# ankitkumar93/compute-war

Measured on AMD Instinct MI355X. Metric: GB/s ingested (Skein-512 + LZ4, 64 KiB blocks), higher is better.
Workload: dtype u64; 1 GPU; skein512+lz4, 1048576 x 65536 B uniform-random blocks/GPU in HBM; blocks_per_gpu=1048576, block_bytes=65536, parallelism=block-sharded x1, gather-only RCCL

## Files before the change

### compute_war_amd/csrc/cw_api.hip

```cpp

#include <hip/hip_runtime.h>

#include <atomic>
#include <condition_variable>
#include <cstdarg>
#include <cstdio>
#include <cstdlib>
#include <cstring>
#include <deque>
#include <memory>
#include <mutex>
#include <string>
#include <thread>
#include <vector>

#include "../../include/cw_hashcompress.h"
#include "cw_device.h"
#include "stream_scratch.h"

namespace {

thread_local char t_err[512] = "";

int fail(int code, const char *fmt, ...)
// ... 104 lines not shown
            HIP_TRY(hipStreamCreateWithFlags(&stream, hipStreamNonBlocking));
        }
        HIP_TRY(side.open(cw::SideStream::least, borrowed ? lender->side.stream : nullptr));
        HIP_TRY(hipEventCreateWithFlags(&ev_meta, hipEventDisableTiming));
        HIP_TRY(hipEventCreateWithFlags(&ev_payload, hipEventDisableTiming));
        HIP_TRY(hipEventCreateWithFlags(&ev_h2d, hipEventDisableTiming));
        return CW_OK;
    }
    void release()
    {
        src.release(); dst.release(); pack.release(); sizes.release(); offs.release(); dig.release();
        h_src.release(); h_meta.release(); h_pack.release();
        if (stream && !borrowed) { cw::release_stream_workspaces(stream); (void)hipStreamDestroy(stream); }
        if (side.stream && !side.borrowed) cw::release_stream_workspaces(side.stream);
        side.release();
        borrowed = false;
        if (ev_meta) (void)hipEventDestroy(ev_meta);
        if (ev_payload) (void)hipEventDestroy(ev_payload);
        if (ev_h2d) (void)hipEventDestroy(ev_h2d);
        stream = nullptr; ev_meta = ev_payload = ev_h2d = nullptr;
    }
};

struct FusedHint { uint32_t *h_queued = nullptr; hipEvent_t ev = nullptr; bool pending = false; size_t blocks_of_copy = 0; float queued_share = 0.f; };

struct ThreadCtx {
    int device = -1;
    FusedHint hint;
    hipStream_t stream = nullptr;
    hipStream_t s_h2d = nullptr, s_d2h = nullptr;
    cw::SideStream side;
    DevBuf src, dst, dig, sizes;
    Slot slot[kSlots];
    int open(int dev)
    {
        if (stream) return CW_OK;
        device = dev;
        HIP_TRY(hipSetDevice(dev));
        HIP_TRY(hipStreamCreateWithFlags(&stream, hipStreamNonBlocking));
        HIP_TRY(hipStreamCreateWithFlags(&s_h2d, hipStreamNonBlocking));
        HIP_TRY(hipStreamCreateWithFlags(&s_d2h, hipStreamNonBlocking));
        HIP_TRY(side.open(cw::SideStream::least));
        return CW_OK;
    }
    ~ThreadCtx()
    {
        if (!stream) return;
        (void)hipSetDevice(device);
        src.release(); dst.release(); dig.release(); sizes.release();
        for (Slot &s : slot) s.release();
        if (hint.ev) (void)hipEventDestroy(hint.ev);
        if (hint.h_queued) (void)hipHostFree(hint.h_queued);
        cw::release_stream_workspaces(side.stream); cw::release_stream_workspaces(stream);
        side.release();
        (void)hipStreamDestroy(s_h2d); (void)hipStreamDestroy(s_d2h); (void)hipStreamDestroy(stream);
    }
};
struct ThreadCtxSet { std::unique_ptr<ThreadCtx> of[kMaxDevices]; };
thread_local ThreadCtxSet t_ctxs;

int thread_ctx(ThreadCtx **out)
{
    int rc = ensure_init();
    if (rc != CW_OK) return rc;
    const int d = current_device();
    std::unique_ptr<ThreadCtx> &c = t_ctxs.of[d];
    if (!c) c.reset(new ThreadCtx);
    if ((rc = c->open(d)) != CW_OK) return rc;
    *out = c.get();
    return CW_OK;
}

const size_t kMaxChunkBytes = (size_t)256 << 20;

// ... 58 lines not shown
void positive(int &f, const char *v) { if (atoi(v) > 0) f = atoi(v); }
void positive(long &f, const char *v) { if (atol(v) > 0) f = atol(v); }

struct KnobDef { const char *name; void (*decode)(Knobs &k, const char *v); };
const KnobDef kKnobTable[] = {
    {"CW_SKEIN_SLICED", [](Knobs &k, const char *v) { k.skein_sliced = v[0] != '0'; }},
    {"CW_LZ4_LANES_FP", [](Knobs &k, const char *v) { k.lz4_lanes_fp = v[0] != '0'; }},
    {"CW_LZF_STHREAD", [](Knobs &k, const char *v) { k.lzf_sthread = v[0] != '0'; }},
    {"CW_SERIAL", [](Knobs &k, const char *v) { k.serial = v[0] == '1'; }},
    {"CW_DEBUG_HOST", [](Knobs &k, const char *v) { k.debug_host = v[0] == '1'; }},
    {"CW_PREPARE_COLD", [](Knobs &k, const char *v) { k.prepare_cold = v[0] == '1'; }},
    {"CW_FUSED_GATE", [](Knobs &k, const char *v) { k.fused_gate = v[0] == '1'; }},
    {"CW_HOST_SHARED_STREAMS", [](Knobs &k, const char *v) { k.host_shared_streams = v[0] == '1'; }},
    {"CW_LANES_CONCURRENT", [](Knobs &k, const char *v) { k.lanes_concurrent = v[0] != '0'; }},
    {"CW_SIDE_PRIO", [](Knobs &k, const char *v) { k.side_prio = v[0] == '0' ? cw::SidePrio::none : v[0] == '2' ? cw::SidePrio::both : cw::SidePrio::lanes; }},
    {"CW_LZ4_MODE", [](Knobs &k, const char *v) {
         k.lz4_mode = !strcmp(v, "scan") ? cw::Lz4Mode::scan : !strcmp(v, "generic") ? cw::Lz4Mode::generic
                    : !strcmp(v, "stream") ? cw::Lz4Mode::stream : !strcmp(v, "cut") ? cw::Lz4Mode::cut : cw::Lz4Mode::normal; }},
    {"CW_LZF_MODE", [](Knobs &k, const char *v) { k.lzf_mode = !strcmp(v, "cut") ? cw::LzfMode::cut : !strcmp(v, "table") ? cw::LzfMode::table : cw::LzfMode::normal; }},
    {"CW_SKEIN_MODE", [](Knobs &k, const char *v) { k.skein_mode = !strcmp(v, "steps") ? cw::SkeinMode::steps : cw::SkeinMode::lines; }},
    {"CW_LZ4_PARSE", [](Knobs &k, const char *v) { k.lz4_parse_fp = !strcmp(v, "fp"); }},
    {"CW_DEBUG_LZF", [](Knobs &k, const char *) { k.debug_lzf = true; }},
    {"CW_SCAN_WPC", [](Knobs &k, const char *v) { positive(k.scan_wpc, v); }},
    {"CW_PARSE_WPC", [](Knobs &k, const char *v) { positive(k.parse_wpc, v); }},
    {"CW_LANES_WPC", [](Knobs &k, const char *v) { positive(k.lanes_wpc, v); }},
    {"CW_LANES_RESERVE", [](Knobs &k, const char *v) { positive(k.lanes_reserve, v); }},
    {"CW_VTAB_WPC", [](Knobs &k, const char *v) { positive(k.vtab_wpc, v); }},
    {"CW_LZF_ST_WPC", [](Knobs &k, const char *v) { positive(k.lzf_st_wpc, v); }},
    {"CW_LZF_ROUND", [](Knobs &k, const char *v) { positive(k.lzf_round, v); }},
    {"CW_LZF_LDS_MAX", [](Knobs &k, const char *v) { positive(k.lzf_lds_max, v); }},
    {"CW_SKEIN_NSLICES", [](Knobs &k, const char *v) { positive(k.skein_nslices, v); }},
    {"CW_HOST_CHUNK_MB", [](Knobs &k, const char *v) { positive(k.host_chunk_mb, v); }},
    {"CW_HOST_BIG_CHUNK_MB", [](Knobs &k, const char *v) { positive(k.host_big_chunk_mb, v); }},
    {"CW_CDC_SEGMENT", [](Knobs &k, const char *v) { positive(k.cdc_segment, v); }},
    {"CW_LZ_FORCE_REDO", [](Knobs &k, const char *v) { k.force_redo = atoi(v) > 0; }},
    {"CW_LZF_SHARE_GIVE_UP", [](Knobs &k, const char *v) { k.lzf_share_give_up = atoi(v) > 0; }},
    {"CW_LZ4_LANES", [](Knobs &k, const char *v) { k.lz4_lanes = atoi(v); }},
    {"CW_LZF_LANES", [](Knobs &k, const char *v) { k.lzf_lanes = atoi(v); }},
    {"CW_DECODE_LANES", [](Knobs &k, const char *v) { k.decode_lanes = atoi(v); }},
    {"CW_LANES_LEAVE", [](Knobs &k, const char *v) { k.lanes_leave = atoi(v); }},
    {"CW_VTAB_MIN", [](Knobs &k, const char *v) { k.vtab_min = atoi(v); }},
    {"CW_VTAB_MAX", [](Knobs &k, const char *v) { k.vtab_max = atoi(v); }},
    {"CW_VTAB_RESERVE", [](Knobs &k, const char *v) { k.vtab_reserve = atoi(v); }},
    {"CW_LZ4_VTAB", [](Knobs &k, const char *v) { k.lz4_vtab = atoi(v); }},
    {"CW_LZ4_LANES_RING", [](Knobs &k, const char *v) { k.lz4_lanes_ring = atoi(v); }},
    {"CW_LZ4_HEADW", [](Knobs &k, const char *v) { k.lz4_headw = atoi(v); }},
// ... 174 lines not shown
    const hipStream_t side = side_s.stream;
    struct Gate { int hash_alg; const uint8_t *src; size_t bb, stride, n; uint8_t *dig; hipStream_t side; cw::SideStream::Fork *fork; int rc; bool called; };
    Gate gate = {hash_alg, d_src, block_bytes, src_stride, nblocks, d_digests, side, &fork, CW_OK, false};
    const cw::AfterScan hook = {[](void *p) -> hipError_t {
                                    Gate *g = static_cast<Gate *>(p);
                                    g->called = true;
                                    g->rc = dev_hash(g->hash_alg, g->src, g->bb, g->stride, g->n, g->dig, g->side, false, true);
                                    return g->rc != CW_OK ? hipErrorUnknown : g->fork->join();
                                }, &gate};
    ThreadCtx *tc = nullptr;
    FusedHint *hint = comp_alg == CW_COMP_LZ4 && thread_ctx(&tc) == CW_OK ? &tc->hint : nullptr;
    if (hint && hint->pending) {
        const hipError_t q = hipEventQuery(hint->ev);
        if (q == hipSuccess) {
            hint->pending = false;
            if (hint->blocks_of_copy) hint->queued_share = (float)*hint->h_queued / (float)hint->blocks_of_copy;
        } else if (q == hipErrorNotReady) {
            (void)hipGetLastError();
        }
    }
    const bool gated = hint && (kn.fused_gate ? *kn.fused_gate : block_bytes <= 4096 && nblocks >= 16384 && hint->queued_share >= 0.25f);
    rc = dev_compress(comp_alg, d_src, block_bytes, src_stride, nblocks, d_dst, dst_stride, d_sizes, main_s, gated ? &hook : nullptr);
    if (gate.called && gate.rc != CW_OK) return gate.rc;
    if (rc == CW_OK && !gate.called) rc = dev_hash(hash_alg, d_src, block_bytes, src_stride, nblocks, d_digests, side, false, true);
    HIP_TRY(fork.join());
    if (rc == CW_OK && hint && !hint->pending) {
        const uint32_t *word = cw::lz4_queued_blocks_word(main_s);
        if (word) {
            if (!hint->h_queued) HIP_TRY(hipHostMalloc(reinterpret_cast<void **>(&hint->h_queued), 64, hipHostMallocDefault));
            if (!hint->ev) HIP_TRY(hipEventCreateWithFlags(&hint->ev, hipEventDisableTiming));
            HIP_TRY(hipMemcpyAsync(hint->h_queued, word, sizeof(uint32_t), hipMemcpyDeviceToHost, main_s));
            HIP_TRY(hipEventRecord(hint->ev, main_s));
            hint->pending = true;
            hint->blocks_of_copy = nblocks;
        }
    }
    return rc;
}

int cw_dev_hash_and_compress(int hash_alg, int comp_alg, const void *d_src, size_t block_bytes, size_t src_stride,
                             size_t nblocks, void *d_digests, void *d_dst, size_t dst_stride, uint32_t *d_sizes, void *stream)
{
    if (comp_alg == CW_COMP_NONE) return cw_dev_hash(hash_alg, d_src, block_bytes, src_stride, nblocks, d_digests, stream);
    if (hash_alg == CW_HASH_NONE)
        return cw_dev_compress(comp_alg, d_src, block_bytes, src_stride, nblocks, d_dst, dst_stride, d_sizes, stream);
    ThreadCtx *c;
    int rc = thread_ctx(&c);
    if (rc != CW_OK) return rc;
    if (nblocks == 0) return CW_OK;
    if (!d_src || !d_dst || !d_sizes || !d_digests) return fail(CW_ERR_BAD_ARG, "NULL device pointer");
    if ((rc = check_block(block_bytes)) != CW_OK) return rc;
    if (src_stride < block_bytes) return fail(CW_ERR_BAD_ARG, "src_stride < block_bytes");
    return dev_fused(c->side, hash_alg, comp_alg, (const uint8_t *)d_src, block_bytes, src_stride, nblocks, (uint8_t *)d_digests, (uint8_t *)d_dst,
                     dst_stride, d_sizes, (hipStream_t)stream);
}

int cw_dev_decompress(int comp_alg, const void *d_comp, size_t comp_stride, const uint32_t *d_sizes, size_t nblocks, void *d_dst,
                      size_t block_bytes, uint32_t *d_status, void *stream)
{
// ... 87 lines not shown
    return CW_OK;
}
int cw_dev_download(void *dst, const void *d_src, size_t bytes)
{
    int rc = ensure_init();
    if (rc != CW_OK) return rc;
    HIP_TRY(hipMemcpy(dst, d_src, bytes, hipMemcpyDeviceToHost));
    return CW_OK;
}
int cw_dev_synchronize(void)
{
    int rc = ensure_init();
    if (rc != CW_OK) return rc;
    HIP_TRY(hipDeviceSynchronize());
    return CW_OK;
}

#ifdef CW_CLOCK_STAMP
int cw_debug_clock_read(int which, unsigned long long *out)
{
    int rc = ensure_init();
    if (rc != CW_OK) return rc;
    HIP_TRY(hipDeviceSynchronize());
    HIP_TRY(which == 0 ? cw::skein_clock_read(out) : cw::lz4_clock_read(out));
    return CW_OK;
}
#endif

void cw_profile_enable(int on) { t_prof_on = on != 0; }

int cw_profile_read(double ms_sum[3], unsigned count[3], int reset)
{
    for (int k = 0; k < PROF_KINDS; k++) { ms_sum[k] = 0; count[k] = 0; }
    for (ProfSpan &p : t_prof) {
        float ms = 0;
        HIP_TRY(hipEventSynchronize(p.b));
        HIP_TRY(hipEventElapsedTime(&ms, p.a, p.b));
        ms_sum[p.kind] += ms;
        count[p.kind]++;
    }
    if (reset) {
        for (ProfSpan &p : t_prof) { (void)hipEventDestroy(p.a); (void)hipEventDestroy(p.b); }
        t_prof.clear();
    }
    return CW_OK;
}

// ... 1102 lines not shown
```

### compute_war_amd/csrc/cw_device.h

```cpp
#pragma once

#include <hip/hip_runtime.h>
#include <stddef.h>
#include <stdint.h>

#include <optional>

#ifndef CW_SKEIN_THREADS
#define CW_SKEIN_THREADS 64
#endif

namespace cw {

#ifdef CW_CLOCK_STAMP
constexpr unsigned kClockSlots = 1024;
struct ClockScope {
    unsigned long long m0 = 0, r0 = 0;
    unsigned long long *rec;
    bool on;
    __device__ ClockScope(unsigned long long *buf, unsigned wg) : rec(buf + 4 * (wg % kClockSlots)), on(threadIdx.x == 0)
    {
        if (on) { m0 = __builtin_amdgcn_s_memtime(); r0 = __builtin_amdgcn_s_memrealtime(); }
    }
    __device__ ~ClockScope()
    {
        if (on) {
            const unsigned long long m1 = __builtin_amdgcn_s_memtime(), r1 = __builtin_amdgcn_s_memrealtime();
            rec[0] = m0; rec[1] = r0; rec[2] = m1; rec[3] = r1;
        }
    }
};
#define CW_CLOCK_SCOPE(buf) ClockScope clock_scope_(buf, blockIdx.x)
#define CW_CLOCK_SCOPE_KEYED(buf, key) ClockScope clock_scope_(buf, ((unsigned)(key) % 8u) * 128u + blockIdx.x % 128u)
hipError_t skein_clock_read(unsigned long long *out);
hipError_t lz4_clock_read(unsigned long long *out);
#else
#define CW_CLOCK_SCOPE(buf) do { } while (0)
#define CW_CLOCK_SCOPE_KEYED(buf, key) do { } while (0)
#endif

struct SkeinIV { uint64_t w[8]; };

void note_kernels(int kind, const char *names);
enum class Lz4Mode : uint8_t { normal, scan, generic, stream, cut };
enum class LzfMode : uint8_t { normal, cut, table };
enum class SkeinMode : uint8_t { by_lean, steps, lines };
enum class SidePrio : uint8_t { both, lanes, none };
struct Knobs {
    bool skein_sliced = true, lz4_lanes_fp = true, lzf_sthread = true;
    bool serial = false, debug_host = false, prepare_cold = false;
    std::optional<bool> fused_gate, host_shared_streams;
    std::optional<bool> lanes_concurrent;
    SidePrio side_prio = SidePrio::both;
    Lz4Mode lz4_mode = Lz4Mode::normal;
    LzfMode lzf_mode = LzfMode::normal;
    SkeinMode skein_mode = SkeinMode::by_lean;
    bool lz4_parse_fp = false;
    bool debug_lzf = false;
    int scan_wpc = 0, parse_wpc = 0, lanes_wpc = 0, lanes_reserve = 0, vtab_wpc = 0, lzf_st_wpc = 0, lzf_round = 0, lzf_lds_max = 0,
        skein_nslices = 0;
    long host_chunk_mb = 0, host_big_chunk_mb = 0, cdc_segment = 0;
    bool force_redo = false, lzf_share_give_up = false;
    std::optional<int> lz4_lanes, lzf_lanes, decode_lanes, lanes_leave, vtab_min, vtab_max, vtab_reserve, lz4_vtab, lz4_lanes_ring,
        lz4_headw, lz4_ltab, vtab_gen;
    std::optional<int> lz4_stage_max;
};
Knobs knobs();

void skein_compute_iv(int state_words, unsigned hash_bits, SkeinIV *iv, uint64_t tree_info = 0);
bool skein_sliced_applies(int state_words, const uint8_t *src, size_t block_bytes, size_t src_stride, size_t nblocks,
                          const uint8_t *digests);
hipError_t skein_sliced_launch(int state_words, const uint8_t *src, size_t block_bytes, size_t src_stride, size_t nblocks, const SkeinIV &iv,
                               uint8_t *digests, unsigned digest_bytes, hipStream_t stream);
hipError_t skein_tree_launch(int state_words, const uint8_t *src, size_t block_bytes, size_t src_stride, size_t nblocks,
                             unsigned hash_bits, unsigned leaf, unsigned node, unsigned max_level, uint8_t *digests, hipStream_t stream);

hipError_t skein512_launch(const uint8_t *src, size_t block_bytes, size_t src_stride, size_t nblocks, const SkeinIV &iv,
                           uint8_t *digests, unsigned digest_bytes, hipStream_t stream, bool lean = false);
hipError_t skein256_launch(const uint8_t *src, size_t block_bytes, size_t src_stride, size_t nblocks, const SkeinIV &iv,
                           uint8_t *digests, unsigned digest_bytes, hipStream_t stream, bool lean = false);
hipError_t sha256_launch(const uint8_t *src, size_t block_bytes, size_t src_stride, size_t nblocks, uint8_t *digests,
                         hipStream_t stream);
// ... 89 lines not shown
```

### compute_war_amd/csrc/lz4_kernel.hip

```cpp

#include <hip/hip_runtime.h>
#include <stdint.h>
#include <stdio.h>
#include <stdlib.h>
#include <string.h>

#include <type_traits>

#include "cw_device.h"
#include "lane_codec.h"
#include "lz_device.h"
#include "stream_scratch.h"

#ifndef HEADW_GLOBAL
#define HEADW_GLOBAL 16
#endif
#ifndef HEADW_STAGED
#define HEADW_STAGED 64
#endif

namespace cw {

using lz::Around;
using lz::around;
// ... 422 lines not shown
    w.qnext = q + 1;
}

__device__ __forceinline__ void probe_range(SpanWalk &w, uint32_t qe, uint32_t *tab, const uint32_t *ring32, uint32_t tag, const uint8_t *g,
                                            uint32_t lane)
{
    uint32_t q = w.qnext;
    w.qnext = qe;
    uint32_t p = __umul24(q, lane) + group_base(q);
    for (; q + 2 <= qe; q += 2) {
        const uint32_t pos[2] = {p, p + lane + (64 * q + 1)};
        if (probe_batches<2, false>(pos, 0, 64, tab, ring32, tag, w.v0, g, lane)) { w.marked = true; return; }
        p = pos[1] + lane + (64 * q + 65);
    }
    if (q < qe) {
        const uint32_t pos[1] = {p};
        w.marked = probe_batches<1, false>(pos, 0, 64, tab, ring32, tag, w.v0, g, lane);
    }
}

#ifdef CW_CLOCK_STAMP
__device__ unsigned long long g_clock_scan[4 * kClockSlots];
hipError_t lz4_clock_read(unsigned long long *out) { return hipMemcpyFromSymbol(out, HIP_SYMBOL(g_clock_scan), sizeof g_clock_scan); }
#endif

template <bool ALIGNED>
__global__ void __launch_bounds__(64)
lz4_scan_span_kernel(const uint8_t *__restrict__ src, uint32_t n, size_t src_stride, uint32_t nspans, uint8_t *__restrict__ dst,
                     size_t dst_stride, uint32_t *__restrict__ sizes, uint32_t nprobes, uint32_t *__restrict__ queue,
                     uint32_t *__restrict__ counters, uint32_t lg)
{
    CW_CLOCK_SCOPE(g_clock_scan);
    __shared__ __attribute__((aligned(16))) uint32_t tab[1u << 13];
    __shared__ __attribute__((aligned(16))) uint32_t ring32[kRing / 4];
    volatile uint32_t *mailbox = ring32;
    const uint32_t lane = threadIdx.x;
    __builtin_amdgcn_s_setprio(3);
    uint32_t epoch = 15;
    const uint32_t cmask = (1u << lg) - 1, run = 16u >> lg;
    const uint32_t hdr = 1 + (n - 15) / 255 + 1;
    const uint32_t lane16 = lane * 16;
    const uint32_t qlast = (nprobes + 61) >> 6;
    const uint32_t gend = group_end((lane + 1) * kChunk < n ? (lane + 1) * kChunk : n, qlast);
    const uint32_t hdrw = (0xFFu << 16) | (((n - 15) % 255) << 24);

    for (;;) {
        __syncthreads();
        if (lane == 0) *mailbox = atomicAdd(&counters[2], 1u);
        __syncthreads();
        const uint32_t span = __builtin_amdgcn_readfirstlane(*mailbox);
        if (span >= nspans) break;
        __syncthreads();
        const size_t first = (size_t)span * run;
        const uint8_t *gs = src + first * src_stride;
        uint8_t *os = dst + first * dst_stride + (ALIGNED ? hdr - 2 : hdr);

        SpanWalk w;
        size_t blk = first;
        uint32_t tag = 0, marks = 0;
        Chunk r0, r1, r2;
#define CW_LD(R, I)                                                                                          \
        do {                                                                                                 \
            const uint32_t i_ = (I) < 15u ? (I) : 15u;                                                       \
            const uint8_t *p_ = gs + (size_t)(i_ >> lg) * src_stride + ((i_ & cmask) << 12) + lane16;        \
            _Pragma("unroll") for (uint32_t j = 0; j < kPieces; j++) R.p[j] = *reinterpret_cast<const uint4 *>(p_ + j * 1024); \
        } while (0)
#define CW_ST(R, I)                                                                                          \
        do {                                                                                                 \
            const uint32_t i_ = (I), c_ = i_ & cmask;                                                        \
            uint8_t *p_ = os + (size_t)(i_ >> lg) * dst_stride + (c_ << 12) + lane16;                        \
            if constexpr (ALIGNED) {                                                                         \
                const uint32_t b_ = ((c_ & 1u) << 12) + lane16;  \
                uint32_t pw_[kPieces];                                                                       \
                _Pragma("unroll") for (uint32_t j = 0; j < kPieces; j++) pw_[j] = ring32[((b_ + j * 1024 - 4) & (kRing - 4)) / 4]; \
                if (c_ == 0 && lane == 0) pw_[0] = hdrw;                                                     \
                _Pragma("unroll") for (uint32_t j = 0; j < kPieces; j++) {                                   \
                    store16_nt(p_ + j * 1024, __builtin_amdgcn_alignbyte(R.p[j].x, pw_[j], 2),               \
                               __builtin_amdgcn_alignbyte(R.p[j].y, R.p[j].x, 2),                            \
                               __builtin_amdgcn_alignbyte(R.p[j].z, R.p[j].y, 2),                            \
                               __builtin_amdgcn_alignbyte(R.p[j].w, R.p[j].z, 2));                           \
                }                                                                                            \
                if (c_ == cmask && lane == 63)                                 \
                    *reinterpret_cast<uint16_t *>(p_ + (kPieces - 1) * 1024 + 16) = (uint16_t)(R.p[kPieces - 1].w >> 16); \
            } else {                                                                                         \
                _Pragma("unroll") for (uint32_t j = 0; j < kPieces; j++) {                                   \
                    uint32_t *q = reinterpret_cast<uint32_t *>(p_ + j * 1024);  \
                    __builtin_nontemporal_store(R.p[j].x, q);     __builtin_nontemporal_store(R.p[j].y, q + 1); \
                    __builtin_nontemporal_store(R.p[j].z, q + 2); __builtin_nontemporal_store(R.p[j].w, q + 3); \
                }                                                                                            \
            }                                                                                                \
        } while (0)
#define CW_FINISH()                                                                                          \
        do {  \
            if (nprobes && !w.marked) probe_partial(w, qlast, nprobes, tab, ring32, tag, src + blk * src_stride, lane); \
            if (w.marked) marks |= 1u << (uint32_t)(blk - first);         \
            else {                                                                                           \
                uint8_t *out = dst + blk * dst_stride;                                                       \
                if constexpr (ALIGNED) {                                                                     \
                    if (lane < (hdr - 2) / 16)                                                               \
                        store16_nt(out + lane16, lane ? ~0u : 0xFFFFFFF0u, ~0u, ~0u, ~0u);                   \
                } else {                                                                                     \
                    if (lane == 0) out[0] = 15u << 4;                                                        \
                    put_len(out + 1, n - 15, lane);                                                          \
                }                                                                                            \
                if (lane == 0) sizes[blk] = hdr + n;                                                         \
            }                                                                                                \
        } while (0)
#define CW_BEGIN(I)                                                                                          \
        do {                                                                                                 \
            blk = first + ((I) >> lg);                                                                       \
            scan_begin_block(tab, epoch, lane);                                                              \
            tag = epoch << 28;                                                                               \
            w = SpanWalk();                                                                                  \
        } while (0)
#define CW_STAGE_IN(R, C)                                                                                    \
        do {                                                                                                 \
            uint8_t *p_ = reinterpret_cast<uint8_t *>(ring32) + (((C) & 1u) << 12) + lane16;                 \
            _Pragma("unroll") for (uint32_t j = 0; j < kPieces; j++) *reinterpret_cast<uint4 *>(p_ + j * 1024) = R.p[j]; \
        } while (0)
#define CW_AFTER_STAGE(C)                                                                                    \
        do {                                                                                                 \
            if ((C) == 0) {                                                                                  \
                w.v0 = ring32[0];                                                                            \
                if (nprobes && lane == 0) {                                                                  \
                    const uint32_t h0 = w.v0 * 2654435761u;                                                  \
                    atomicMax(&tab[h0 >> 19], tag | ((h0 >> 7) & 0xFFFu));                   \
                }                                                                                            \
                if (qlast) probe_partial(w, 0u, nprobes, tab, ring32, tag, src + blk * src_stride, lane);    \
            }                                                                                                \
            if (!w.marked) probe_range(w, __builtin_amdgcn_readlane(gend, (C)), tab, ring32, tag, src + blk * src_stride, lane); \
        } while (0)
#define CW_STEP(PREV, CUR, I)                                                                                \
        do {                                                                                                 \
            const uint32_t s_ = (I), c_ = s_ & cmask;                                                        \
            CW_ST(PREV, s_ - 1);                                                                             \
            CW_LD(PREV, s_ + 2);                                                                             \
            if (c_ == 0) { CW_FINISH(); CW_BEGIN(s_); }                                                      \
            CW_STAGE_IN(CUR, c_);                                                                            \
            CW_AFTER_STAGE(c_);                                                                              \
        } while (0)

        CW_LD(r0, 0u);
        CW_LD(r1, 1u);
        CW_LD(r2, 2u);
        CW_BEGIN(0u);
        CW_STAGE_IN(r0, 0u);
        CW_AFTER_STAGE(0u);
        for (uint32_t i = 1; i < 16; i += 3) {
            CW_STEP(r0, r1, i);
            CW_STEP(r1, r2, i + 1);
            CW_STEP(r2, r0, i + 2);
        }
        CW_ST(r0, 15u);
        CW_FINISH();
        if (marks) {
            uint32_t base = 0;
            if (lane == 0) base = atomicAdd(&counters[1], (uint32_t)__builtin_popcount(marks));
            base = __builtin_amdgcn_readfirstlane(base);
            if (lane < 16 && ((marks >> lane) & 1u)) {
                sizes[first + lane] = kNeedsParse;
                queue[base + (uint32_t)__builtin_popcount(marks & ((1u << lane) - 1u))] = (uint32_t)(first + lane);
            }
        }
#undef CW_LD
#undef CW_ST
#undef CW_FINISH
#undef CW_BEGIN
#undef CW_STAGE_IN
#undef CW_AFTER_STAGE
#undef CW_STEP
    }
}

static uint32_t scan_probes(uint32_t n)
{
    if (n < kMFLimit + 1) return 0;
    const uint32_t limit = n - 11;
    uint32_t k = 0, p = 1, step = 1, nb = 64;
    while (p + step <= limit) { p += step; step = nb++ >> 6; k++; }
    return k;
}

template <bool STAGED>
__global__ void __launch_bounds__(64)
lz4_blocks_kernel(const uint8_t *__restrict__ src, uint32_t n, size_t src_stride, size_t nblocks,
                  uint8_t *__restrict__ dst, size_t dst_stride, uint32_t *__restrict__ sizes,
                  const uint32_t *__restrict__ queue, uint32_t *__restrict__ counters)
{
    extern __shared__ __attribute__((aligned(16))) uint8_t smem[];
    uint16_t *tab = reinterpret_cast<uint16_t *>(smem);
    uint8_t *lds_in = smem + kTabBytes;
    const uint32_t lane = threadIdx.x;

    const uint32_t qcount = counters[1];
// ... 1085 lines not shown
    std::optional<SideStream::Fork> lanes_fork, vtab_fork;
    char launched[320] = "";
    auto note = [&](const char *fmt, auto... a) __attribute__((format(printf, 2, 0))) {
        const size_t used = strlen(launched);
        if (used && used + 3 < sizeof launched) strcat(launched, " + ");
        const size_t at = strlen(launched);
#pragma clang diagnostic push
#pragma clang diagnostic ignored "-Wformat-security"
        snprintf(launched + at, sizeof launched - at, fmt, a...);
#pragma clang diagnostic pop
    };

    if ((e = hipMemsetAsync(counters, 0, 8 * sizeof(uint32_t), stream)) != hipSuccess) return e;
    const size_t scan_grid = nblocks < 256 * 5 ? nblocks : 256 * 5;
    const bool streamable = ((reinterpret_cast<uintptr_t>(src) | src_stride | n) & 15) == 0 && kn.lz4_mode != Lz4Mode::generic;
    if (streamable) {
        const size_t wpc = kn.scan_wpc ? (size_t)kn.scan_wpc : 4;
        const bool pow2 = n >= kChunk && (n & (n - 1)) == 0 && kn.lz4_mode != Lz4Mode::stream;
        uint32_t lg = 0;
        while (pow2 && (kChunk << lg) < n) lg++;
        const size_t run = pow2 ? (size_t)(16u >> lg) : 1;
        const size_t nspans = pow2 ? nblocks / run : 0, done = nspans * run;
        if (nspans) {
            const size_t g = nspans < 256 * wpc ? nspans : 256 * wpc;
            const bool aligned = ((reinterpret_cast<uintptr_t>(dst) | dst_stride) & 15) == 0;
            if (aligned) {
                hipLaunchKernelGGL(lz4_scan_span_kernel<true>, dim3((unsigned)g), dim3(64), 0, stream, src, n, src_stride, (uint32_t)nspans,
                                   dst, dst_stride, sizes, scan_probes(n), queue, counters, lg);
                note("cw::lz4_scan_span_kernel<true>");
            } else {
                hipLaunchKernelGGL(lz4_scan_span_kernel<false>, dim3((unsigned)g), dim3(64), 0, stream, src, n, src_stride, (uint32_t)nspans,
                                   dst, dst_stride, sizes, scan_probes(n), queue, counters, lg);
                note("cw::lz4_scan_span_kernel<false>");
            }
        }
        if (done < nblocks) {
            const size_t rest = nblocks - done;
            const size_t sgrid = rest < 256 * wpc ? rest : 256 * wpc;
            hipLaunchKernelGGL(lz4_scan_stream_kernel, dim3((unsigned)sgrid), dim3(64), 0, stream, src, n, src_stride, nblocks, dst,
                               dst_stride, sizes, scan_probes(n), queue, counters, done, 3u);
            note("cw::lz4_scan_stream_kernel");
        }
    } else {
        hipLaunchKernelGGL(lz4_scan_kernel, dim3((unsigned)scan_grid), dim3(64), 0, stream, src, n, src_stride, nblocks, dst,
                           dst_stride, sizes, scan_probes(n), queue, counters);
        note("cw::lz4_scan_kernel");
    }
// ... 147 lines not shown
```

### compute_war_amd/csrc/misc_kernels.hip

```cpp

#include <hip/hip_runtime.h>
#include <stdint.h>

#include "cw_device.h"

namespace cw {

static __device__ __forceinline__ uint64_t splitmix64(uint64_t x)
{
    uint64_t z = x + 0x9E3779B97F4A7C15ULL;
    z = (z ^ (z >> 30)) * 0xBF58476D1CE4E5B9ULL;
    z = (z ^ (z >> 27)) * 0x94D049BB133111EBULL;
    return z ^ (z >> 31);
}

__global__ void __launch_bounds__(256)
gen_random_kernel(uint64_t seed, uint64_t first_block, size_t total_pairs, unsigned pairs_per_block, uint4 *__restrict__ dst)
{
    const size_t stride = (size_t)gridDim.x * blockDim.x;
    for (size_t i = (size_t)blockIdx.x * blockDim.x + threadIdx.x; i < total_pairs; i += stride) {
        const uint64_t blk = first_block + i / pairs_per_block;
        const uint64_t w = 2 * (i % pairs_per_block);
        const uint64_t a = splitmix64(seed ^ ((blk << 13) | w));
        const uint64_t b = splitmix64(seed ^ ((blk << 13) | (w + 1)));
// ... 35 lines not shown
    size_t grid = (total + 255) / 256;
    if (grid > 256 * 16) grid = 256 * 16;
    hipLaunchKernelGGL(gen_mixed_kernel, dim3((unsigned)grid), dim3(256), 0, stream, seed, first_block, total,
                       (unsigned)(block_bytes / 16), reinterpret_cast<uint4 *>(dst));
    return hipGetLastError();
}

hipError_t gen_random_launch(uint64_t seed, uint64_t first_block, size_t nblocks, size_t block_bytes, uint8_t *dst,
                             hipStream_t stream)
{
    if (nblocks == 0 || block_bytes == 0) return hipSuccess;
    if (block_bytes % 16 || (reinterpret_cast<uintptr_t>(dst) & 15)) return hipErrorInvalidValue;
    const size_t total = nblocks * (block_bytes / 16);
    size_t grid = (total + 255) / 256;
    if (grid > 256 * 16) grid = 256 * 16;
    hipLaunchKernelGGL(gen_random_kernel, dim3((unsigned)grid), dim3(256), 0, stream, seed, first_block, total,
                       (unsigned)(block_bytes / 16), reinterpret_cast<uint4 *>(dst));
    return hipGetLastError();
}

__global__ void __launch_bounds__(256)
sum_sizes_kernel(const uint32_t *__restrict__ sizes, size_t n, uint32_t raw_bytes, unsigned long long *__restrict__ totals)
{
    unsigned long long bytes = 0, zeros = 0;
    const size_t stride = (size_t)gridDim.x * blockDim.x;
    for (size_t i = (size_t)blockIdx.x * blockDim.x + threadIdx.x; i < n; i += stride) {
        const uint32_t s = sizes[i];
        bytes += s ? s : raw_bytes;
        zeros += s == 0;
    }
    for (int off = 32; off > 0; off >>= 1) {
        bytes += __shfl_down(bytes, off, 64);
        zeros += __shfl_down(zeros, off, 64);
    }
    if ((threadIdx.x & 63) == 0) {
        atomicAdd(&totals[0], bytes);
        atomicAdd(&totals[1], zeros);
    }
}

hipError_t sum_sizes_launch(const uint32_t *sizes, size_t n, uint32_t raw_bytes, uint64_t *totals, hipStream_t stream)
{
    if (n == 0) return hipSuccess;
    size_t grid = (n + 255) / 256;
    if (grid > 1024) grid = 1024;
    hipLaunchKernelGGL(sum_sizes_kernel, dim3((unsigned)grid), dim3(256), 0, stream, sizes, n, raw_bytes,
                       reinterpret_cast<unsigned long long *>(totals));
    return hipGetLastError();
}

}
```

Before: 1132 GB/s.

## Prefetch next LZ4 scan span across iterations and move hint copy off main stream

The LZ4 scan-span kernel is restructured into one continuous software pipeline. It pulls the next span index early with an atomic and preloads its first chunks while the current span finishes, which removes the per-span syncthreads/mailbox handoff and the pipeline drain and refill. The queued-blocks hint readback now runs on a separate copy stream gated by an event, so it no longer serializes on the main stream behind the join. sum_sizes is unrolled with an LDS block reduction and a smaller grid to cut atomics. It also adds a scan-grid knob and clock-stamp instrumentation. The risks are more complex control flow with a replay path at the tail and higher register pressure.

```diff
diff --git a/compute_war_amd/csrc/cw_api.hip b/compute_war_amd/csrc/cw_api.hip
--- a/compute_war_amd/csrc/cw_api.hip
+++ b/compute_war_amd/csrc/cw_api.hip
@@ -150,7 +150,14 @@
     }
 };
 
-struct FusedHint { uint32_t *h_queued = nullptr; hipEvent_t ev = nullptr; bool pending = false; size_t blocks_of_copy = 0; float queued_share = 0.f; };
+struct FusedHint {
+    uint32_t *h_queued = nullptr;
+    hipEvent_t ev = nullptr, ev_codec = nullptr;
+    hipStream_t copy_s = nullptr;
+    bool pending = false;
+    size_t blocks_of_copy = 0;
+    float queued_share = 0.f;
+};
 
 struct ThreadCtx {
     int device = -1;
@@ -178,6 +185,8 @@
         src.release(); dst.release(); dig.release(); sizes.release();
         for (Slot &s : slot) s.release();
         if (hint.ev) (void)hipEventDestroy(hint.ev);
+        if (hint.ev_codec) (void)hipEventDestroy(hint.ev_codec);
+        if (hint.copy_s) (void)hipStreamDestroy(hint.copy_s);
         if (hint.h_queued) (void)hipHostFree(hint.h_queued);
         cw::release_stream_workspaces(side.stream); cw::release_stream_workspaces(stream);
         side.release();
@@ -282,6 +291,7 @@
     {"CW_LZ4_PARSE", [](Knobs &k, const char *v) { k.lz4_parse_fp = !strcmp(v, "fp"); }},
     {"CW_DEBUG_LZF", [](Knobs &k, const char *) { k.debug_lzf = true; }},
     {"CW_SCAN_WPC", [](Knobs &k, const char *v) { positive(k.scan_wpc, v); }},
+    {"CW_SCAN_GRID", [](Knobs &k, const char *v) { positive(k.scan_grid, v); }},
     {"CW_PARSE_WPC", [](Knobs &k, const char *v) { positive(k.parse_wpc, v); }},
     {"CW_LANES_WPC", [](Knobs &k, const char *v) { positive(k.lanes_wpc, v); }},
     {"CW_LANES_RESERVE", [](Knobs &k, const char *v) { positive(k.lanes_reserve, v); }},
@@ -502,19 +512,24 @@
     const bool gated = hint && (kn.fused_gate ? *kn.fused_gate : block_bytes <= 4096 && nblocks >= 16384 && hint->queued_share >= 0.25f);
     rc = dev_compress(comp_alg, d_src, block_bytes, src_stride, nblocks, d_dst, dst_stride, d_sizes, main_s, gated ? &hook : nullptr);
     if (gate.called && gate.rc != CW_OK) return gate.rc;
+    const uint32_t *word = rc == CW_OK && hint && !hint->pending ? cw::lz4_queued_blocks_word(main_s) : nullptr;
+    if (word) {
+        if (!hint->h_queued) HIP_TRY(hipHostMalloc(reinterpret_cast<void **>(&hint->h_queued), 64, hipHostMallocDefault));
+        if (!hint->ev) HIP_TRY(hipEventCreateWithFlags(&hint->ev, hipEventDisableTiming));
+        if (!hint->ev_codec) HIP_TRY(hipEventCreateWithFlags(&hint->ev_codec, hipEventDisableTiming));
+        if (!hint->copy_s) HIP_TRY(hipStreamCreateWithFlags(&hint->copy_s, hipStreamNonBlocking));
+        HIP_TRY(hipEventRecord(hint->ev_codec, main_s));
+    }
     if (rc == CW_OK && !gate.called) rc = dev_hash(hash_alg, d_src, block_bytes, src_stride, nblocks, d_digests, side, false, true);
+    if (word) {
+        HIP_TRY(hipStreamWaitEvent(hint->copy_s, hint->ev_codec, 0));
+        HIP_TRY(hipMemcpyAsync(hint->h_queued, word, sizeof(uint32_t), hipMemcpyDeviceToHost, hint->copy_s));
+        HIP_TRY(hipEventRecord(hint->ev, hint->copy_s));
+        HIP_TRY(hipStreamWaitEvent(main_s, hint->ev, 0));
+        hint->pending = true;
+        hint->blocks_of_copy = nblocks;
+    }
     HIP_TRY(fork.join());
-    if (rc == CW_OK && hint && !hint->pending) {
-        const uint32_t *word = cw::lz4_queued_blocks_word(main_s);
-        if (word) {
-            if (!hint->h_queued) HIP_TRY(hipHostMalloc(reinterpret_cast<void **>(&hint->h_queued), 64, hipHostMallocDefault));
-            if (!hint->ev) HIP_TRY(hipEventCreateWithFlags(&hint->ev, hipEventDisableTiming));
-            HIP_TRY(hipMemcpyAsync(hint->h_queued, word, sizeof(uint32_t), hipMemcpyDeviceToHost, main_s));
-            HIP_TRY(hipEventRecord(hint->ev, main_s));
-            hint->pending = true;
-            hint->blocks_of_copy = nblocks;
-        }
-    }
     return rc;
 }
 
@@ -648,7 +663,7 @@
     int rc = ensure_init();
     if (rc != CW_OK) return rc;
     HIP_TRY(hipDeviceSynchronize());
-    HIP_TRY(which == 0 ? cw::skein_clock_read(out) : cw::lz4_clock_read(out));
+    HIP_TRY(which == 0 ? cw::skein_clock_read(out) : which == 2 ? cw::lz4_span_stamp_read(out) : cw::lz4_clock_read(out));
     return CW_OK;
 }
 #endif
diff --git a/compute_war_amd/csrc/cw_device.h b/compute_war_amd/csrc/cw_device.h
--- a/compute_war_amd/csrc/cw_device.h
+++ b/compute_war_amd/csrc/cw_device.h
@@ -34,6 +34,7 @@
 #define CW_CLOCK_SCOPE_KEYED(buf, key) ClockScope clock_scope_(buf, ((unsigned)(key) % 8u) * 128u + blockIdx.x % 128u)
 hipError_t skein_clock_read(unsigned long long *out);
 hipError_t lz4_clock_read(unsigned long long *out);
+hipError_t lz4_span_stamp_read(unsigned long long *out);
 #else
 #define CW_CLOCK_SCOPE(buf) do { } while (0)
 #define CW_CLOCK_SCOPE_KEYED(buf, key) do { } while (0)
@@ -57,7 +58,7 @@
     SkeinMode skein_mode = SkeinMode::by_lean;
     bool lz4_parse_fp = false;
     bool debug_lzf = false;
-    int scan_wpc = 0, parse_wpc = 0, lanes_wpc = 0, lanes_reserve = 0, vtab_wpc = 0, lzf_st_wpc = 0, lzf_round = 0, lzf_lds_max = 0,
+    int scan_wpc = 0, scan_grid = 0, parse_wpc = 0, lanes_wpc = 0, lanes_reserve = 0, vtab_wpc = 0, lzf_st_wpc = 0, lzf_round = 0, lzf_lds_max = 0,
         skein_nslices = 0;
     long host_chunk_mb = 0, host_big_chunk_mb = 0, cdc_segment = 0;
     bool force_redo = false, lzf_share_give_up = false;
diff --git a/compute_war_amd/csrc/lz4_kernel.hip b/compute_war_amd/csrc/lz4_kernel.hip
--- a/compute_war_amd/csrc/lz4_kernel.hip
+++ b/compute_war_amd/csrc/lz4_kernel.hip
@@ -468,6 +468,30 @@
 #ifdef CW_CLOCK_STAMP
 __device__ unsigned long long g_clock_scan[4 * kClockSlots];
 hipError_t lz4_clock_read(unsigned long long *out) { return hipMemcpyFromSymbol(out, HIP_SYMBOL(g_clock_scan), sizeof g_clock_scan); }
+__device__ unsigned long long g_span_stamp[4 * kClockSlots];
+hipError_t lz4_span_stamp_read(unsigned long long *out) { return hipMemcpyFromSymbol(out, HIP_SYMBOL(g_span_stamp), sizeof g_span_stamp); }
+struct SpanStamp {
+    unsigned long long t0 = 0, head = 0, whole = 0, spans = 0;
+    __device__ void at(int i)
+    {
+        const unsigned long long t = __builtin_amdgcn_s_memtime();
+        if (i == 1) head += t - t0;
+        if (i == 2) {
+            whole += t - t0;
+            spans++;
+            if (threadIdx.x == 0) {
+                unsigned long long *rec = g_span_stamp + 4 * (blockIdx.x % kClockSlots);
+                rec[0] = head; rec[1] = whole; rec[2] = spans; rec[3] = 0;
+            }
+        }
+        if (i != 1) t0 = t;
+    }
+};
+#define CW_SPAN_STAMP_DECL SpanStamp span_stamp_
+#define CW_SPAN_STAMP(i) span_stamp_.at(i)
+#else
+#define CW_SPAN_STAMP_DECL do { } while (0)
+#define CW_SPAN_STAMP(i) do { } while (0)
 #endif
 
 template <bool ALIGNED>
@@ -479,7 +503,6 @@
     CW_CLOCK_SCOPE(g_clock_scan);
     __shared__ __attribute__((aligned(16))) uint32_t tab[1u << 13];
     __shared__ __attribute__((aligned(16))) uint32_t ring32[kRing / 4];
-    volatile uint32_t *mailbox = ring32;
     const uint32_t lane = threadIdx.x;
     __builtin_amdgcn_s_setprio(3);
     uint32_t epoch = 15;
@@ -490,132 +513,156 @@
     const uint32_t gend = group_end((lane + 1) * kChunk < n ? (lane + 1) * kChunk : n, qlast);
     const uint32_t hdrw = (0xFFu << 16) | (((n - 15) % 255) << 24);
 
-    for (;;) {
-        __syncthreads();
-        if (lane == 0) *mailbox = atomicAdd(&counters[2], 1u);
-        __syncthreads();
-        const uint32_t span = __builtin_amdgcn_readfirstlane(*mailbox);
-        if (span >= nspans) break;
-        __syncthreads();
-        const size_t first = (size_t)span * run;
-        const uint8_t *gs = src + first * src_stride;
-        uint8_t *os = dst + first * dst_stride + (ALIGNED ? hdr - 2 : hdr);
-
-        SpanWalk w;
-        size_t blk = first;
-        uint32_t tag = 0, marks = 0;
-        Chunk r0, r1, r2;
+    uint32_t pull_at = 2;
+    asm volatile("" : "+v"(pull_at));
+    uint32_t pulled = 0;
+    if (lane == 0) pulled = atomicAdd(&counters[pull_at], 1u);
+    const uint32_t span0 = __builtin_amdgcn_readfirstlane(pulled);
+    if (span0 >= nspans) return;
+    size_t first = (size_t)span0 * run, blk = first;
+    const uint8_t *gs = src + first * src_stride, *gn = gs;
+    uint8_t *os = dst + first * dst_stride + (ALIGNED ? hdr - 2 : hdr);
+    uint32_t next = ~0u;
+    bool replay = false;
+    SpanWalk w;
+    uint32_t tag = 0, marks = 0;
+    Chunk r0, r1, r2;
+    CW_SPAN_STAMP_DECL;
+    CW_SPAN_STAMP(0);
 #define CW_LD(R, I)                                                                                          \
-        do {                                                                                                 \
-            const uint32_t i_ = (I) < 15u ? (I) : 15u;                                                       \
-            const uint8_t *p_ = gs + (size_t)(i_ >> lg) * src_stride + ((i_ & cmask) << 12) + lane16;        \
-            _Pragma("unroll") for (uint32_t j = 0; j < kPieces; j++) R.p[j] = *reinterpret_cast<const uint4 *>(p_ + j * 1024); \
-        } while (0)
+    do {                         \
+        const uint32_t l_ = (I), i_ = l_ & 15u;                                                              \
+        const uint8_t *p_ = (l_ < 16u ? gs : gn) + (size_t)(i_ >> lg) * src_stride + ((i_ & cmask) << 12) + lane16; \
+        _Pragma("unroll") for (uint32_t j = 0; j < kPieces; j++) R.p[j] = *reinterpret_cast<const uint4 *>(p_ + j * 1024); \
+    } while (0)
 #define CW_ST(R, I)                                                                                          \
-        do {                                                                                                 \
-            const uint32_t i_ = (I), c_ = i_ & cmask;                                                        \
-            uint8_t *p_ = os + (size_t)(i_ >> lg) * dst_stride + (c_ << 12) + lane16;                        \
+    do {                                                                                                     \
+        const uint32_t i_ = (I), c_ = i_ & cmask;                                                            \
+        uint8_t *p_ = os + (size_t)(i_ >> lg) * dst_stride + (c_ << 12) + lane16;                            \
+        if constexpr (ALIGNED) {                                                                             \
+            const uint32_t b_ = ((c_ & 1u) << 12) + lane16;  \
+            uint32_t pw_[kPieces];                                                                           \
+            _Pragma("unroll") for (uint32_t j = 0; j < kPieces; j++) pw_[j] = ring32[((b_ + j * 1024 - 4) & (kRing - 4)) / 4]; \
+            if (c_ == 0 && lane == 0) pw_[0] = hdrw;                                                         \
+            _Pragma("unroll") for (uint32_t j = 0; j < kPieces; j++) {                                       \
+                store16_nt(p_ + j * 1024, __builtin_amdgcn_alignbyte(R.p[j].x, pw_[j], 2),                   \
+                           __builtin_amdgcn_alignbyte(R.p[j].y, R.p[j].x, 2),                                \
+                           __builtin_amdgcn_alignbyte(R.p[j].z, R.p[j].y, 2),                                \
+                           __builtin_amdgcn_alignbyte(R.p[j].w, R.p[j].z, 2));                               \
+            }                                                                                                \
+            if (c_ == cmask && lane == 63)                                     \
+                *reinterpret_cast<uint16_t *>(p_ + (kPieces - 1) * 1024 + 16) = (uint16_t)(R.p[kPieces - 1].w >> 16); \
+        } else {                                                                                             \
+            _Pragma("unroll") for (uint32_t j = 0; j < kPieces; j++) {                                       \
+                uint32_t *q = reinterpret_cast<uint32_t *>(p_ + j * 1024);  \
+                __builtin_nontemporal_store(R.p[j].x, q);     __builtin_nontemporal_store(R.p[j].y, q + 1);  \
+                __builtin_nontemporal_store(R.p[j].z, q + 2); __builtin_nontemporal_store(R.p[j].w, q + 3);  \
+            }                                                                                                \
+        }                                                                                                    \
+    } while (0)
+#define CW_FINISH()                                                                                          \
+    do {  \
+        if (nprobes && !w.marked) probe_partial(w, qlast, nprobes, tab, ring32, tag, src + blk * src_stride, lane); \
+        if (w.marked) marks |= 1u << (uint32_t)(blk - first);             \
+        else {                                                                                               \
+            uint8_t *out = dst + blk * dst_stride;                                                           \
             if constexpr (ALIGNED) {                                                                         \
-                const uint32_t b_ = ((c_ & 1u) << 12) + lane16;  \
-                uint32_t pw_[kPieces];                                                                       \
-                _Pragma("unroll") for (uint32_t j = 0; j < kPieces; j++) pw_[j] = ring32[((b_ + j * 1024 - 4) & (kRing - 4)) / 4]; \
-                if (c_ == 0 && lane == 0) pw_[0] = hdrw;                                                     \
-                _Pragma("unroll") for (uint32_t j = 0; j < kPieces; j++) {                                   \
-                    store16_nt(p_ + j * 1024, __builtin_amdgcn_alignbyte(R.p[j].x, pw_[j], 2),               \
-                               __builtin_amdgcn_alignbyte(R.p[j].y, R.p[j].x, 2),                            \
-                               __builtin_amdgcn_alignbyte(R.p[j].z, R.p[j].y, 2),                            \
-                               __builtin_amdgcn_alignbyte(R.p[j].w, R.p[j].z, 2));                           \
-                }                                                                                            \
-                if (c_ == cmask && lane == 63)                                 \
-                    *reinterpret_cast<uint16_t *>(p_ + (kPieces - 1) * 1024 + 16) = (uint16_t)(R.p[kPieces - 1].w >> 16); \
+                if (lane < (hdr - 2) / 16)                                                                   \
+                    store16_nt(out + lane16, lane ? ~0u : 0xFFFFFFF0u, ~0u, ~0u, ~0u);                       \
             } else {                                                                                         \
-                _Pragma("unroll") for (uint32_t j = 0; j < kPieces; j++) {                                   \
-                    uint32_t *q = reinterpret_cast<uint32_t *>(p_ + j * 1024);  \
-                    __builtin_nontemporal_store(R.p[j].x, q);     __builtin_nontemporal_store(R.p[j].y, q + 1); \
-                    __builtin_nontemporal_store(R.p[j].z, q + 2); __builtin_nontemporal_store(R.p[j].w, q + 3); \
-                }                                                                                            \
+                if (lane == 0) out[0] = 15u << 4;                                                            \
+                put_len(out + 1, n - 15, lane);                                                              \
             }                                                                                                \
-        } while (0)
-#define CW_FINISH()                                                                                          \
-        do {  \
-            if (nprobes && !w.marked) probe_partial(w, qlast, nprobes, tab, ring32, tag, src + blk * src_stride, lane); \
-            if (w.marked) marks |= 1u << (uint32_t)(blk - first);         \
-            else {                                                                                           \
-                uint8_t *out = dst + blk * dst_stride;                                                       \
-                if constexpr (ALIGNED) {                                                                     \
-                    if (lane < (hdr - 2) / 16)                                                               \
-                        store16_nt(out + lane16, lane ? ~0u : 0xFFFFFFF0u, ~0u, ~0u, ~0u);                   \
-                } else {                                                                                     \
-                    if (lane == 0) out[0] = 15u << 4;                                                        \
-                    put_len(out + 1, n - 15, lane);                                                          \
-                }                                                                                            \
-                if (lane == 0) sizes[blk] = hdr + n;                                                         \
+            if (lane == 0) sizes[blk] = hdr + n;                                                             \
+        }                                                                                                    \
+    } while (0)
+#define CW_QUEUE_MARKS()                                                                                     \
+    do {                                                                                                     \
+        if (marks) {                                                                                         \
+            uint32_t base = 0;                                                                               \
+            if (lane == 0) base = atomicAdd(&counters[1], (uint32_t)__builtin_popcount(marks));  \
+            base = __builtin_amdgcn_readfirstlane(base);                                                     \
+            if (lane < 16 && ((marks >> lane) & 1u)) {                                                       \
+                sizes[first + lane] = kNeedsParse;                                                           \
+                queue[base + (uint32_t)__builtin_popcount(marks & ((1u << lane) - 1u))] = (uint32_t)(first + lane); \
             }                                                                                                \
-        } while (0)
+        }                                                                                                    \
+    } while (0)
 #define CW_BEGIN(I)                                                                                          \
-        do {                                                                                                 \
-            blk = first + ((I) >> lg);                                                                       \
-            scan_begin_block(tab, epoch, lane);                                                              \
-            tag = epoch << 28;                                                                               \
-            w = SpanWalk();                                                                                  \
-        } while (0)
+    do {                                                                                                     \
+        blk = first + ((I) >> lg);                                                                           \
+        scan_begin_block(tab, epoch, lane);                                                                  \
+        tag = epoch << 28;                                                                                   \
+        w = SpanWalk();                                                                                      \
+    } while (0)
 #define CW_STAGE_IN(R, C)                                                                                    \
-        do {                                                                                                 \
-            uint8_t *p_ = reinterpret_cast<uint8_t *>(ring32) + (((C) & 1u) << 12) + lane16;                 \
-            _Pragma("unroll") for (uint32_t j = 0; j < kPieces; j++) *reinterpret_cast<uint4 *>(p_ + j * 1024) = R.p[j]; \
-        } while (0)
+    do {                                                                                                     \
+        uint8_t *p_ = reinterpret_cast<uint8_t *>(ring32) + (((C) & 1u) << 12) + lane16;                     \
+        _Pragma("unroll") for (uint32_t j = 0; j < kPieces; j++) *reinterpret_cast<uint4 *>(p_ + j * 1024) = R.p[j]; \
+    } while (0)
 #define CW_AFTER_STAGE(C)                                                                                    \
-        do {                                                                                                 \
-            if ((C) == 0) {                                                                                  \
-                w.v0 = ring32[0];                                                                            \
-                if (nprobes && lane == 0) {                                                                  \
-                    const uint32_t h0 = w.v0 * 2654435761u;                                                  \
-                    atomicMax(&tab[h0 >> 19], tag | ((h0 >> 7) & 0xFFFu));                   \
-                }                                                                                            \
-                if (qlast) probe_partial(w, 0u, nprobes, tab, ring32, tag, src + blk * src_stride, lane);    \
+    do {                                                                                                     \
+        if ((C) == 0) {                                                                                      \
+            w.v0 = ring32[0];                                                                                \
+            if (nprobes && lane == 0) {                                                                      \
+                const uint32_t h0 = w.v0 * 2654435761u;                                                      \
+                atomicMax(&tab[h0 >> 19], tag | ((h0 >> 7) & 0xFFFu));                       \
             }                                                                                                \
-            if (!w.marked) probe_range(w, __builtin_amdgcn_readlane(gend, (C)), tab, ring32, tag, src + blk * src_stride, lane); \
-        } while (0)
-#define CW_STEP(PREV, CUR, I)                                                                                \
-        do {                                                                                                 \
-            const uint32_t s_ = (I), c_ = s_ & cmask;                                                        \
-            CW_ST(PREV, s_ - 1);                                                                             \
-            CW_LD(PREV, s_ + 2);                                                                             \
-            if (c_ == 0) { CW_FINISH(); CW_BEGIN(s_); }                                                      \
-            CW_STAGE_IN(CUR, c_);                                                                            \
-            CW_AFTER_STAGE(c_);                                                                              \
-        } while (0)
-
-        CW_LD(r0, 0u);
-        CW_LD(r1, 1u);
-        CW_LD(r2, 2u);
-        CW_BEGIN(0u);
-        CW_STAGE_IN(r0, 0u);
-        CW_AFTER_STAGE(0u);
-        for (uint32_t i = 1; i < 16; i += 3) {
-            CW_STEP(r0, r1, i);
-            CW_STEP(r1, r2, i + 1);
-            CW_STEP(r2, r0, i + 2);
-        }
-        CW_ST(r0, 15u);
-        CW_FINISH();
-        if (marks) {
-            uint32_t base = 0;
-            if (lane == 0) base = atomicAdd(&counters[1], (uint32_t)__builtin_popcount(marks));
-            base = __builtin_amdgcn_readfirstlane(base);
-            if (lane < 16 && ((marks >> lane) & 1u)) {
-                sizes[first + lane] = kNeedsParse;
-                queue[base + (uint32_t)__builtin_popcount(marks & ((1u << lane) - 1u))] = (uint32_t)(first + lane);
-            }
-        }
+            if (qlast) probe_partial(w, 0u, nprobes, tab, ring32, tag, src + blk * src_stride, lane);        \
+        }                                                                                                    \
+        if (!w.marked) probe_range(w, __builtin_amdgcn_readlane(gend, (C)), tab, ring32, tag, src + blk * src_stride, lane); \
+    } while (0)
+#define CW_STEP(PREV, CUR, K)                                                                                \
+    {                                                                                                        \
+        const uint32_t c_ = s & cmask;                                                                       \
+        CW_ST(PREV, (s - 1u) & 15u);                                                                         \
+        if ((K) == 0 && s - 10u <= 2u && lane == 0) pulled = atomicAdd(&counters[pull_at], 1u);              \
+        if ((K) == 2 && s - 12u <= 2u) {                                                                     \
+            next = __builtin_amdgcn_readfirstlane(pulled);                                                   \
+            gn = next < nspans ? src + (size_t)next * run * src_stride : gs;                                 \
+        }                                                                                                    \
+        gs = s == 0u ? gn : gs;                                                                              \
+        CW_LD(PREV, s + 2u);                                                                                 \
+        if (c_ == 0) {                                                                                       \
+            if (!replay) CW_FINISH();                                                                        \
+            if (s == 0u) {                                                                                   \
+                CW_QUEUE_MARKS();                                                                            \
+                CW_SPAN_STAMP(2);                                                                            \
+                replay = next >= nspans;                                                                     \
+                first = replay ? first : (size_t)next * run;                                                 \
+                os = dst + first * dst_stride + (ALIGNED ? hdr - 2 : hdr);                                   \
+                marks = 0;                                                                                   \
+                next = ~0u;                                                                                  \
+            }                                                                                                \
+            CW_BEGIN(s);                                                                                     \
+        }                                                                                                    \
+        CW_STAGE_IN(CUR, c_);                                                                                \
+        if (s == 0u) CW_SPAN_STAMP(1);                                                                       \
+        CW_AFTER_STAGE(c_);                                                                                  \
+        s = (s + 1u) & 15u;                                                                                  \
+    }
+
+    CW_LD(r0, 0u);
+    CW_LD(r1, 1u);
+    CW_LD(r2, 2u);
+    CW_BEGIN(0u);
+    CW_STAGE_IN(r0, 0u);
+    CW_SPAN_STAMP(1);
+    CW_AFTER_STAGE(0u);
+    uint32_t s = 1;
+    do {
+        CW_STEP(r0, r1, 0)
+        CW_STEP(r1, r2, 1)
+        CW_STEP(r2, r0, 2)
+    } while (!replay);
 #undef CW_LD
 #undef CW_ST
 #undef CW_FINISH
+#undef CW_QUEUE_MARKS
 #undef CW_BEGIN
 #undef CW_STAGE_IN
 #undef CW_AFTER_STAGE
 #undef CW_STEP
-    }
 }
 
 static uint32_t scan_probes(uint32_t n)
@@ -1747,7 +1794,8 @@
         const size_t run = pow2 ? (size_t)(16u >> lg) : 1;
         const size_t nspans = pow2 ? nblocks / run : 0, done = nspans * run;
         if (nspans) {
-            const size_t g = nspans < 256 * wpc ? nspans : 256 * wpc;
+            const size_t gmax = kn.scan_grid ? (size_t)kn.scan_grid : 256 * wpc;
+            const size_t g = nspans < gmax ? nspans : gmax;
             const bool aligned = ((reinterpret_cast<uintptr_t>(dst) | dst_stride) & 15) == 0;
             if (aligned) {
                 hipLaunchKernelGGL(lz4_scan_span_kernel<true>, dim3((unsigned)g), dim3(64), 0, stream, src, n, src_stride, (uint32_t)nspans,
diff --git a/compute_war_amd/csrc/misc_kernels.hip b/compute_war_amd/csrc/misc_kernels.hip
--- a/compute_war_amd/csrc/misc_kernels.hip
+++ b/compute_war_amd/csrc/misc_kernels.hip
@@ -81,9 +81,21 @@
 __global__ void __launch_bounds__(256)
 sum_sizes_kernel(const uint32_t *__restrict__ sizes, size_t n, uint32_t raw_bytes, unsigned long long *__restrict__ totals)
 {
+    __shared__ unsigned long long part[2][4];
     unsigned long long bytes = 0, zeros = 0;
     const size_t stride = (size_t)gridDim.x * blockDim.x;
-    for (size_t i = (size_t)blockIdx.x * blockDim.x + threadIdx.x; i < n; i += stride) {
+    size_t i = (size_t)blockIdx.x * blockDim.x + threadIdx.x;
+    for (; i + 3 * stride < n; i += 4 * stride) {
+        uint32_t s[4];
+#pragma unroll
+        for (int k = 0; k < 4; k++) s[k] = sizes[i + k * stride];
+#pragma unroll
+        for (int k = 0; k < 4; k++) {
+            bytes += s[k] ? s[k] : raw_bytes;
+            zeros += s[k] == 0;
+        }
+    }
+    for (; i < n; i += stride) {
         const uint32_t s = sizes[i];
         bytes += s ? s : raw_bytes;
         zeros += s == 0;
@@ -93,8 +105,13 @@
         zeros += __shfl_down(zeros, off, 64);
     }
     if ((threadIdx.x & 63) == 0) {
-        atomicAdd(&totals[0], bytes);
-        atomicAdd(&totals[1], zeros);
+        part[0][threadIdx.x >> 6] = bytes;
+        part[1][threadIdx.x >> 6] = zeros;
+    }
+    __syncthreads();
+    if (threadIdx.x < 2) {
+        const unsigned long long *p = part[threadIdx.x];
+        atomicAdd(&totals[threadIdx.x], p[0] + p[1] + p[2] + p[3]);
     }
 }
 
@@ -102,7 +119,7 @@
 {
     if (n == 0) return hipSuccess;
     size_t grid = (n + 255) / 256;
-    if (grid > 1024) grid = 1024;
+    if (grid > 256) grid = 256;
     hipLaunchKernelGGL(sum_sizes_kernel, dim3((unsigned)grid), dim3(256), 0, stream, sizes, n, raw_bytes,
                        reinterpret_cast<unsigned long long *>(totals));
     return hipGetLastError();
```

Measured after the change: 1136 GB/s (median of 5 runs). About the same (+0.4%).
